# Kitware/SMQTK-Indexing

Hardware: AMD Instinct MI355X
Metric: queries/sec, exact brute-force l2 kNN k=100 over 10000000x128 float32 (recall@100 = 1.0 by construction); scan HBM GB/s vs 8 TB/s peak (higher is better)
Workload: dtype f32 results (distances bit-identical to numpy float32); filter arithmetic int8 MFMA (i32 accumulation, measured per-row error bound), exact re-rank f32

## Files before the change

### smqtk_indexing_amd/csrc/sq_dense_i8.hpp

```cpp
#pragma once
#include "sq_dense_i8_policy.hpp"
#include "sq_dense_scan.hpp"

namespace sq {

typedef int i32x4 __attribute__((ext_vector_type(4)));
typedef int i32x16 __attribute__((ext_vector_type(16)));

template <int KS>
struct I8Geom {
    static constexpr int ROW_BYTES = KS * 32;
    static constexpr int UNIT_ROWS = KS == 4 ? 64 : 32;
    static constexpr int TILES = UNIT_ROWS / 32;
    static constexpr int UNIT_BYTES = UNIT_ROWS * ROW_BYTES;
    static constexpr int SLOT_BYTES = UNIT_BYTES + 256;
    static constexpr int WAVES = KS <= 8 ? 8 : 4;
    static constexpr int NSTAGE = 2;
    static constexpr int PIECES = UNIT_BYTES / 1024;
    static constexpr int SAMPLES_PER_UNIT = 2 * TILES;
};
static constexpr int I8_MAX_ROW_BYTES = 512;
__host__ __device__ constexpr int i8_row_bytes(int d) { return d <= 128 ? 128 : (d <= 256 ? 256 : 512); }
__host__ __device__ constexpr int i8_unit_rows(int row_bytes) { return row_bytes == 128 ? 64 : 32; }

// ... 101 lines not shown
                                                                   const double* __restrict__ nx64, float inv_dx, float dx,
                                                                   signed char* __restrict__ out8, float* __restrict__ nrow,
                                                                   float* __restrict__ r2row, long long row_base, int row_bytes) {
    const int lane = threadIdx.x & 63;
    const long long row = row_base + (long long)blockIdx.x * 4 + (threadIdx.x >> 6);
    if (row >= n_pad) return;
    double e2 = 0.0, r2 = 0.0;
    bool finite = true;
    const double inv_norm = (row < n && nx64) ? 1.0 / sqrt(nx64[row]) : 1.0;
    for (int k0 = 0; k0 < row_bytes; k0 += 64 * EPL) {
        unsigned char q[EPL];
#pragma unroll
        for (int j = 0; j < EPL; ++j) q[j] = 0;
        if (row < n) {
#pragma unroll
            for (int j = 0; j < EPL; ++j) {
                const int k = k0 + EPL * lane + j;
                if (k < d) {
                    const float v = db[row * ld + k];
                    const float xc = i8_element(v, center, k, nx64 != nullptr, inv_norm);
                    if (!(xc == xc) || !(fabsf(xc) < 3.0e38f)) finite = false;
                    float t = rintf(xc * inv_dx);
                    t = fminf(fmaxf(t, -127.f), 127.f);
                    if (!(t == t)) t = 0.f;
                    q[j] = (unsigned char)(signed char)(int)t;
                    const double res = (double)xc - (double)t * (double)dx;
                    e2 += (double)xc * (double)xc;
                    r2 += res * res;
                }
            }
        }
        if (k0 + EPL * lane >= row_bytes) continue;
        unsigned char* dst = reinterpret_cast<unsigned char*>(out8) + row * row_bytes + k0 + EPL * lane;
        if constexpr (EPL == 2) {
            *reinterpret_cast<unsigned short*>(dst) = (unsigned short)(q[0] | (q[1] << 8));
        } else if constexpr (EPL == 4) {
            *reinterpret_cast<u32*>(dst) = (u32)q[0] | ((u32)q[1] << 8) | ((u32)q[2] << 16) | ((u32)q[3] << 24);
        } else {
            uint2 w;
            w.x = (u32)q[0] | ((u32)q[1] << 8) | ((u32)q[2] << 16) | ((u32)q[3] << 24);
            w.y = (u32)q[4] | ((u32)q[5] << 8) | ((u32)q[6] << 16) | ((u32)q[7] << 24);
            *reinterpret_cast<uint2*>(dst) = w;
        }
    }
    finite = __ballot(!finite) == 0ull;
    for (int o = 32; o > 0; o >>= 1) {
        e2 += __shfl_xor(e2, o);
        r2 += __shfl_xor(r2, o);
    }
    if (lane == 0) {
        float nr = __builtin_inff(), rr = 0.f;
        if (row < n && finite) {
            nr = nx64 ? 0.f : (float)e2;
            if ((double)nr > e2) nr = __uint_as_float(__float_as_uint(nr) - 1u);
            rr = (float)r2;
            if ((double)rr < r2) rr = __uint_as_float(__float_as_uint(rr) + 1u);
        }
        nrow[row] = nr;
        r2row[row] = rr;
    }
}

static __global__ __launch_bounds__(256) void dense8_resid_stats_kernel(const float* __restrict__ r2row, const float* __restrict__ nrow,
                                                                         long long n, double* __restrict__ sum_r2,
                                                                         u32* __restrict__ max_bits) {
    __shared__ double red[4];
    __shared__ float rmax[4], nmax[4];
    double acc = 0.0;
    float m = 0.f, mn = 0.f;
    for (long long i = (long long)blockIdx.x * 256 + threadIdx.x; i < n; i += (long long)gridDim.x * 256) {
        const float nv = nrow[i];
        if (nv < __builtin_inff() && nv > -__builtin_inff()) {
            const float v = r2row[i];
            acc += (double)v;
            m = fmaxf(m, v);
            mn = fmaxf(mn, nv);
        }
    }
    for (int o = 32; o > 0; o >>= 1) {
        acc += __shfl_xor(acc, o);
        m = fmaxf(m, __shfl_xor(m, o));
        mn = fmaxf(mn, __shfl_xor(mn, o));
    }
    if ((threadIdx.x & 63) == 0) {
        red[threadIdx.x >> 6] = acc;
        rmax[threadIdx.x >> 6] = m;
        nmax[threadIdx.x >> 6] = mn;
    }
    __syncthreads();
    if (threadIdx.x == 0) {
        atomicAdd(sum_r2, red[0] + red[1] + red[2] + red[3]);
        atomicMax(max_bits, __float_as_uint(fmaxf(fmaxf(rmax[0], rmax[1]), fmaxf(rmax[2], rmax[3]))));
        atomicMax(max_bits + 1, __float_as_uint(fmaxf(fmaxf(nmax[0], nmax[1]), fmaxf(nmax[2], nmax[3]))));
    }
}

static __global__ __launch_bounds__(256) void dense8_flag_kernel(const float* __restrict__ r2row, float* __restrict__ nrow, long long n,
                                                                  float r2_cut, u32* __restrict__ flagged, long long row_base) {
    const long long i = row_base + (long long)blockIdx.x * 256 + threadIdx.x;
    if (i >= n) return;
    if (nrow[i] < __builtin_inff() && r2row[i] > r2_cut) {
        nrow[i] = -__builtin_inff();
        atomicAdd(flagged, 1u);
    }
}

template <int EPL>
__device__ __forceinline__ void dense8_prep_query_row(const float* __restrict__ qrow, bool real, int d, const float* __restrict__ center,
                                                      double dx, double r_max, double x_max, int cosine,
                                                      signed char* __restrict__ p0, signed char* __restrict__ p1, float2& par_out,
                                                      double& qn2_out) {
    const int l16 = threadIdx.x & 15;
    const float sc = cosine ? -1.f : -2.f;
    float v[EPL][4];
#pragma unroll
    for (int c = 0; c < EPL; ++c)
#pragma unroll
        for (int e = 0; e < 4; ++e) {
            const int t = 64 * c + l16 + 16 * e;
            float raw = 0.f, cen = 0.f;
            if (real && t < d) {
                raw = qrow[t];
                if (center) cen = center[t];
            }
            v[c][e] = (real && t < d) ? (center ? __fsub_rn(raw, cen) : raw) : 0.f;
        }
    auto chunk_sum = [](double x0, double x1, double x2, double x3) __attribute__((always_inline)) {
        double sacc = (x0 + x2) + (x1 + x3);
        for (int o = 8; o > 0; o >>= 1) sacc += __shfl_xor(sacc, o);
        return sacc;
    };
    if (cosine) {
        double nn = 0.0;
#pragma unroll
        for (int c = 0; c < EPL; ++c)
            nn += chunk_sum((double)v[c][0] * (double)v[c][0], (double)v[c][1] * (double)v[c][1], (double)v[c][2] * (double)v[c][2],
                            (double)v[c][3] * (double)v[c][3]);
        const double rn = sqrt(nn);
#pragma unroll
        for (int c = 0; c < EPL; ++c)
#pragma unroll
            for (int e = 0; e < 4; ++e) v[c][e] = (float)((double)v[c][e] / rn);
    }
    double Q = 0.0;
    float mx = 0.f;
#pragma unroll
    for (int c = 0; c < EPL; ++c) {
        Q += chunk_sum((double)v[c][0] * (double)v[c][0], (double)v[c][1] * (double)v[c][1], (double)v[c][2] * (double)v[c][2],
                       (double)v[c][3] * (double)v[c][3]);
#pragma unroll
        for (int e = 0; e < 4; ++e) {
            float m = fabsf(sc * v[c][e]);
            if (!(m == m)) m = __builtin_inff();
            mx = fmaxf(mx, m);
        }
    }
    for (int o = 8; o > 0; o >>= 1) mx = fmaxf(mx, __shfl_xor(mx, o));
    const bool ok = real && mx < 3.0e38f && mx > 0.f;
    const double dq = ok ? (double)mx / 127.0 : 1.0;
    const double inv_dq = 1.0 / dq;
    double r2s = 0.0;
#pragma unroll
    for (int c = 0; c < EPL; ++c) {
        double r2[4];
#pragma unroll
        for (int e = 0; e < 4; ++e) {
            const double w = (double)(sc * v[c][e]);
            const double ws = w * inv_dq;
            float qt8 = 0.f, ql8 = 0.f;
            if (ok) {
                qt8 = fminf(fmaxf(rintf((float)ws), -127.f), 127.f);
                ql8 = fminf(fmaxf(rintf((float)((ws - (double)qt8) * 256.0)), -127.f), 127.f);
            }
            const int t = 64 * c + l16 + 16 * e;
            p0[t] = (signed char)(int)qt8;
            p1[t] = (signed char)(int)ql8;
            const double res = w - ((double)qt8 + (double)ql8 * 0.00390625) * dq;
            r2[e] = res * res;
        }
        r2s += chunk_sum(r2[0], r2[1], r2[2], r2[3]);
    }
    const double rq = sqrt(r2s) * (1.0 + 1e-9);
    const double unit = dx * dq;
    const double xr = x_max + r_max, qn = sqrt(Q), wn = (cosine ? 1.0 : 2.0) * qn;
    double e = r_max * wn + xr * rq + 4.0 * 5.9604644775390625e-08 * (xr * (wn + rq) + x_max * x_max);
    e *= 1.0 + 1e-6;
    float ef = (float)e;
    if ((double)ef < e) ef = __uint_as_float(__float_as_uint(ef) + 1u);
    if (!ok && real) ef = __builtin_inff();
    par_out = make_float2((float)unit, real ? ef : 0.f);
    qn2_out = real ? Q : 0.0;
}

template <int EPL>
static __global__ __launch_bounds__(64) void dense8_prep_queries_kernel(const float* __restrict__ q, int nq, int d,
                                                                         const float* __restrict__ center, double dx, double r_max,
                                                                         double x_max, signed char* __restrict__ qs8,
                                                                         float2* __restrict__ par, double* __restrict__ qn2,
                                                                         float* __restrict__ thr, u32* __restrict__ cnt,
                                                                         u32* __restrict__ oflag, float* __restrict__ q_al, int ldq,
                                                                         const DenseCallPtrs* __restrict__ ind, int cosine, int plane_rows) {
    constexpr int row_bytes = EPL * 64;
    if (ind) q = ind->q;
    const int qi = blockIdx.x * 4 + (threadIdx.x >> 4), t = threadIdx.x & 15;
    if (t == 0) {
        thr[qi] = qi < nq ? -__builtin_inff() : __builtin_nanf("");
        cnt[qi] = 0u;
        if (qi == 0) *oflag = 0u;
    }
    if (qi < nq)
        for (int i = t; i < ldq; i += 16) q_al[(long long)qi * ldq + i] = i < d ? q[(long long)qi * d + i] : 0.f;
    float2 pr;
    double Q;
    dense8_prep_query_row<EPL>(q + (long long)qi * d, qi < nq, d, center, dx, r_max, x_max, cosine,
                               qs8 + (long long)qi * row_bytes, qs8 + (long long)(plane_rows + qi) * row_bytes, pr, Q);
    if (t == 0) {
        par[qi] = pr;
        qn2[qi] = Q;
    }
}

struct Dense8ThrPost {
    const float2* par;
    const double* qn2;
    __device__ __forceinline__ void prologue(int, double*) const {}
    __device__ __forceinline__ float operator()(int q, float t) const {
        if (!(t < __builtin_inff())) return t;
        if (!(par[q].y < __builtin_inff())) return __builtin_nanf("");
        const double tt = (double)t + 2.0 * (double)par[q].y + 4e-6 * fabs((double)t + qn2[q]);
        float r = (float)tt;
        if ((double)r < tt) r = __uint_as_float(__float_as_uint(r) + (r >= 0.f ? 1 : -1));
        return r;
    }
};

struct Dense8ScanArgs {
    const signed char* scan8;
    const float* nrow;
    long long n;
    long long n_units;
    const signed char* qs8;
    const float2* par;
    const float* thr;
    uint2* wave_out;
    u32* wave_cnt;
    u32 wave_cap;
    float* sample_out;
    long long ns;
    long long unit_step;
    long long n_sel;
    int nrb;
    int nt;
    long long nt_from_row;
    int nqt;
    int plane_rows;
    int debug;
    float* wave_score;
    u32* hist;
};

template <int KS>
__device__ __forceinline__ int i8_swz(int c, int r) {
    if constexpr (KS == 4) return c ^ ((r >> 1) & 7);
    return (c & ~15) | ((c & 15) ^ (r & 15));
}

enum { I8_EMIT = 0, I8_SAMPLE = 1, I8_LANEMIN = 2, I8_EMIT_H = 3 };

static constexpr int I8_HIST_BINS = 64;
static constexpr int I8_CNT_SHIFT = 5;
static constexpr int I8_HIST_WORDS = TILE_ROWS * I8_HIST_BINS + (TILE_ROWS << I8_CNT_SHIFT);

template <int WAVES>
__device__ __forceinline__ void dense8_hist_flush(u32* lds_hist, u32* __restrict__ ghist) {
    constexpr int PER = TILE_ROWS * I8_HIST_BINS / WAVES;
    const int lane = threadIdx.x & 63;
    const int wave = __builtin_amdgcn_readfirstlane(threadIdx.x >> 6);
#pragma unroll
    for (int i = 0; i < PER / 64; ++i) {
        const int b = wave * PER + i * 64 + lane;
        const u32 v = __hip_atomic_exchange(lds_hist + b, 0u, __ATOMIC_RELAXED, __HIP_MEMORY_SCOPE_WORKGROUP);
        if (v) __hip_atomic_fetch_add(ghist + b, v, __ATOMIC_RELAXED, __HIP_MEMORY_SCOPE_AGENT);
    }
}

template <int KS, int MODE>
__device__ __forceinline__ void dense8_stream(const Dense8ScanArgs& a, unsigned char* smem, const i32x4 (&bq)[KS], const i32x4 (&bl)[KS],
                                              float unit_lo, float thr_l, u32& wcount, float& smin, u32* lds_ticket,
                                              float inv_w_l = 0.f, u32* lds_hist = nullptr) {
    using G = I8Geom<KS>;
    constexpr bool SAMPLE = MODE == I8_SAMPLE || MODE == I8_LANEMIN;
    const int lane = threadIdx.x & 63;
    const int wave = __builtin_amdgcn_readfirstlane(threadIdx.x >> 6);
    const int r31 = lane & 31, h = lane >> 5;
    const u32 lds_base = (u32)(uintptr_t)smem;
    const u32 ring_base = lds_base + (u32)wave * (G::NSTAGE * G::SLOT_BYTES);
    const unsigned char* ring_ptr = smem + wave * (G::NSTAGE * G::SLOT_BYTES);
    const long long wave_id = (long long)blockIdx.x * G::WAVES + wave;
    const long long nwaves = (long long)a.nrb * G::WAVES;
    uint2* wout = a.wave_out + wave_id * a.wave_cap;
    float* wsc = MODE == I8_EMIT_H ? a.wave_score + wave_id * a.wave_cap : nullptr;
    u32* hist_l = MODE == I8_EMIT_H ? lds_hist + r31 * I8_HIST_BINS : nullptr;

    const long long wg_first = (long long)blockIdx.x * G::WAVES;
    auto take_unit = [&]() __attribute__((always_inline)) -> long long {
        u32 t = 0;
        if (lane == 0) t = __hip_atomic_fetch_add(lds_ticket, 1u, __ATOMIC_RELAXED, __HIP_MEMORY_SCOPE_WORKGROUP);
        t = (u32)__builtin_amdgcn_readfirstlane((int)t);
        const long long u = wg_first + (long long)(t % G::WAVES) + (long long)(t / G::WAVES) * nwaves;
        return u < a.n_sel ? u : -1ll;
    };
    const long long my_units = wave_id < a.n_sel ? (a.n_sel - wave_id + nwaves - 1) / nwaves : 0;
    u32 voff[G::PIECES];
#pragma unroll
    for (int j = 0; j < G::PIECES; ++j) {
        const int lin = j * 1024 + lane * 16;
        const int r = lin / G::ROW_BYTES, cpos = (lin % G::ROW_BYTES) >> 4;
        voff[j] = (u32)(r * G::ROW_BYTES + i8_swz<KS>(cpos, r) * 16);
    }
    const u32 voff_n = (u32)lane * 4u;
    static_assert(G::NSTAGE == 2, "two ring slots: the units in flight are sel_even / sel_odd");
    long long issued = 0, sel_even = -1, sel_odd = -1;
    bool more = true;
    auto issue_next = [&]() __attribute__((always_inline)) {
        if (!more) return;
        const long long sel = take_unit();
        if (sel < 0) {
            more = false;
            return;
        }
        if (issued & 1) sel_odd = sel; else sel_even = sel;
        const long long unit_idx = sel * a.unit_step;
        const long long row0 = unit_idx * G::UNIT_ROWS;
        const u32 dst = ring_base + (u32)(issued % G::NSTAGE) * G::SLOT_BYTES;
        const unsigned char* base = reinterpret_cast<const unsigned char*>(a.scan8) + row0 * G::ROW_BYTES;
#pragma unroll
        for (int j = 0; j < G::PIECES; ++j) {
            if (a.nt && row0 >= a.nt_from_row)
                glds16<true>(base, voff[j], dst + (u32)j * 1024);
            else
                glds16<false>(base, voff[j], dst + (u32)j * 1024);
        }
        glds4(a.nrow + row0, voff_n, dst + G::UNIT_BYTES);
        ++issued;
    };
    for (int p = 0; p < G::NSTAGE; ++p) issue_next();
    const int flush_every = (int)(my_units >> 3) > 0 ? (int)(my_units >> 3) : 1;
    int to_flush = flush_every;

    for (long long it = 0; it < issued; ++it) {
        const long long sel = (it & 1) ? sel_odd : sel_even;
        const long long unit_idx = sel * a.unit_step;
        const long long row0 = unit_idx * G::UNIT_ROWS;
        wait_units_in_flight<G::NSTAGE, G::PIECES + 1>((int)(issued - it - 1));
        const unsigned char* sl = ring_ptr + (it % G::NSTAGE) * G::SLOT_BYTES;
        constexpr int KH = KS == 16 ? 8 : KS;
        i32x4 av[G::TILES][KH];
        f32x4 nr[G::TILES][4];
#pragma unroll
        for (int t = 0; t < G::TILES; ++t) {
            const int r = 32 * t + r31;
#pragma unroll
            for (int s = 0; s < KH; ++s)
                av[t][s] = *reinterpret_cast<const i32x4*>(sl + r * G::ROW_BYTES + i8_swz<KS>(2 * s + h, r) * 16);
#pragma unroll
            for (int c = 0; c < 4; ++c) nr[t][c] = *reinterpret_cast<const f32x4*>(sl + G::UNIT_BYTES + (32 * t + 8 * c + 4 * h) * 4);
        }
        asm volatile("s_waitcnt lgkmcnt(0)" ::: "memory");
        if constexpr (KS != 16) issue_next();
#pragma unroll
        for (int t = 0; t < G::TILES; ++t) {
            i32x16 acc, acl;
#pragma unroll
            for (int i = 0; i < 16; ++i) acc[i] = acl[i] = 0;
#pragma unroll
            for (int s = 0; s < KH; ++s) {
                acc = __builtin_amdgcn_mfma_i32_32x32x32_i8(av[t][s], bq[s], acc, 0, 0, 0);
                acl = __builtin_amdgcn_mfma_i32_32x32x32_i8(av[t][s], bl[s], acl, 0, 0, 0);
            }
            if constexpr (KS == 16) {
#pragma unroll
                for (int s = 0; s < KH; ++s)
                    av[t][s] = *reinterpret_cast<const i32x4*>(sl + r31 * G::ROW_BYTES + i8_swz<KS>(2 * (KH + s) + h, r31) * 16);
                asm volatile("s_waitcnt lgkmcnt(0)" ::: "memory");
                issue_next();
#pragma unroll
                for (int s = 0; s < KH; ++s) {
                    acc = __builtin_amdgcn_mfma_i32_32x32x32_i8(av[t][s], bq[KH + s], acc, 0, 0, 0);
                    acl = __builtin_amdgcn_mfma_i32_32x32x32_i8(av[t][s], bl[KH + s], acl, 0, 0, 0);
                }
            }
            if (a.debug & 1024) {
                if (acc[0] == 0x7fffffff && acl[5] == 0x7ffffffe) wcount += 1;
                continue;
            }
            float sc[16];
#pragma unroll
            for (int i = 0; i < 16; ++i) {
                float nv = nr[t][i >> 2][i & 3];
                if constexpr (SAMPLE) nv = nv == -__builtin_inff() ? __builtin_inff() : nv;
                sc[i] = __fmaf_rn((float)((acc[i] << 8) + acl[i]), unit_lo, nv);
            }
            float m = sc[0];
#pragma unroll
            for (int i = 1; i < 16; ++i) m = fminf(m, sc[i]);
            if constexpr (MODE == I8_LANEMIN) {
                smin = fminf(smin, m);
            } else if constexpr (MODE == I8_SAMPLE) {
                a.sample_out[(long long)r31 * a.ns + sel * G::SAMPLES_PER_UNIT + t * 2 + h] = m;
            } else {
                const u64 hit = __ballot(m <= thr_l);
                if (hit != 0) {
                    u32 mask = 0;
#pragma unroll
                    for (int i = 0; i < 16; ++i) mask |= (sc[i] <= thr_l ? 1u : 0u) << i;
                    const u64 bal = __ballot(mask != 0);
                    if (mask) {
                        const u32 pos = wcount + __builtin_amdgcn_mbcnt_hi((u32)(bal >> 32), __builtin_amdgcn_mbcnt_lo((u32)bal, 0u));
                        if (pos < a.wave_cap) {
                            wout[pos] = make_uint2((u32)(row0 + 32 * t + 4 * h), (mask << 16) | (u32)r31);
                            if constexpr (MODE == I8_EMIT_H) wsc[pos] = m;
                        }
                        if constexpr (MODE == I8_EMIT_H) {
                            if (m > -__builtin_inff()) {
                                const int bin = min((int)((thr_l - m) * inv_w_l), I8_HIST_BINS - 1);
                                __hip_atomic_fetch_add(hist_l + bin, 1u, __ATOMIC_RELAXED, __HIP_MEMORY_SCOPE_WORKGROUP);
                            }
                        }
                    }
                    wcount += (u32)__popcll(bal);
                }
            }
        }
        if constexpr (MODE == I8_EMIT_H) {
            if (--to_flush == 0) {
                to_flush = flush_every;
                dense8_hist_flush<G::WAVES>(lds_hist, a.hist);
            }
        }
    }
}

template <int KS>
__device__ __forceinline__ void dense8_load_planes(const signed char* planes, i32x4 (&bq)[KS], i32x4 (&bl)[KS]) {
    using G = I8Geom<KS>;
    const int lane = threadIdx.x & 63, r31 = lane & 31, h = lane >> 5;
#pragma unroll
    for (int s = 0; s < KS; ++s) {
        bq[s] = *reinterpret_cast<const i32x4*>(planes + r31 * G::ROW_BYTES + (2 * s + h) * 16);
        bl[s] = *reinterpret_cast<const i32x4*>(planes + (TILE_ROWS + r31) * G::ROW_BYTES + (2 * s + h) * 16);
    }
#pragma unroll
    for (int s = 0; s < KS; ++s) asm volatile("" : "+v"(bq[s]), "+v"(bl[s]));
}

template <int KS, bool SAMPLE>
__global__ __launch_bounds__(I8Geom<KS>::WAVES * 64, KS == 16 ? 1 : 2) void dense8_scan_kernel(Dense8ScanArgs a) {
    using G = I8Geom<KS>;
    extern __shared__ __attribute__((aligned(16))) unsigned char smem[];
    const int lane = threadIdx.x & 63;
    const int wave = __builtin_amdgcn_readfirstlane(threadIdx.x >> 6);
    const int r31 = lane & 31;
    i32x4 bq[KS], bl[KS];
    dense8_load_planes<KS>(a.qs8, bq, bl);
    float unit_lo = a.par[r31].x * 0.00390625f;
    float thr_l = SAMPLE ? 0.f : a.thr[r31];
    asm volatile("" : "+v"(unit_lo), "+v"(thr_l));
    u32 wcount = 0;
    float smin = 0.f;
    __shared__ u32 s_unit_ticket;
    if (threadIdx.x == 0) s_unit_ticket = 0u;
    __syncthreads();
    dense8_stream<KS, SAMPLE ? I8_SAMPLE : I8_EMIT>(a, smem, bq, bl, unit_lo, thr_l, wcount, smin, &s_unit_ticket);
    if constexpr (!SAMPLE) {
        if (lane == 0) {
            const long long wave_id = (long long)blockIdx.x * G::WAVES + wave;
            a.wave_cnt[2 * wave_id] = wcount;
            a.wave_cnt[2 * wave_id + 1] = 0u;
        }
    }
}


struct Dense8HeadArgs {
    Dense8ScanArgs s;
    const float* q;
    int nq, d;
    const float* center;
    double dx, r_max, x_max;
    int cosine;
    double* qn2;
    u32* cnt;
    u32* oflag;
    float* q_al;
    int ldq;
    const DenseCallPtrs* ind;
    float* lane_min;
    int keep;
    int kk;
};

template <int VM, int NQ>
__device__ __forceinline__ void wave_kth_smallest(const float* __restrict__ vals, long long stride, int M, int k, float (&out)[NQ]) {
    const int lane = threadIdx.x & 63;
    constexpr u32 KINF = 0xff800000u;
    u32 key[NQ][VM];
    u32 prefix[NQ];
    u32 xall = 0u;
#pragma unroll
    for (int n = 0; n < NQ; ++n) {
        u32 kmin = KINF, kmax = 0u;
#pragma unroll
        for (int j = 0; j < VM; ++j) {
            const int i = j * 64 + lane;
            u32 kv = ordered_f32(vals[n * stride + (i < M ? i : 0)]);
            kv = (i < M && kv < KINF) ? kv : KINF;
            key[n][j] = kv;
            kmin = kv < kmin ? kv : kmin;
            kmax = kv > kmax ? kv : kmax;
        }
        for (int o = 32; o > 0; o >>= 1) {
            const u32 a = (u32)__shfl_xor((int)kmin, o), b = (u32)__shfl_xor((int)kmax, o);
            kmin = a < kmin ? a : kmin;
            kmax = b > kmax ? b : kmax;
        }
        prefix[n] = __builtin_amdgcn_readfirstlane(kmin);
        xall |= __builtin_amdgcn_readfirstlane(kmin ^ kmax);
    }
    if (xall != 0u) {
        const int top = 31 - __clz((int)xall);
#pragma unroll
        for (int n = 0; n < NQ; ++n) prefix[n] &= ~((2u << top) - 1u);
        for (int b = top; b >= 0; --b) {
#pragma unroll
            for (int n = 0; n < NQ; ++n) {
                const u32 cand = prefix[n] | ((1u << b) - 1u);
                u32 c = 0;
#pragma unroll
                for (int j = 0; j < VM; ++j) c += (u32)__popcll(__ballot(key[n][j] <= cand));
                if (c < (u32)k) prefix[n] |= 1u << b;
            }
        }
    }
#pragma unroll
    for (int n = 0; n < NQ; ++n) {
        float r = unordered_f32(prefix[n]);
        if (prefix[n] >= KINF) {
            u32 c = 0;
#pragma unroll
            for (int j = 0; j < VM; ++j) c += (u32)__popcll(__ballot(key[n][j] < KINF));
            if (c < (u32)k) r = __builtin_inff();
        }
        out[n] = r;
    }
}

template <int KS>
__global__ __launch_bounds__(I8Geom<KS>::WAVES * 64, KS == 16 ? 1 : 2) void dense8_head_kernel(Dense8HeadArgs ha) {
    using G = I8Geom<KS>;
    constexpr int VB = G::WAVES * 2;
    extern __shared__ __attribute__((aligned(16))) unsigned char smem[];
    __shared__ float2 s_par[TILE_ROWS];
    __shared__ double s_qn2[TILE_ROWS];
    __shared__ float s_lm[TILE_ROWS][16];
    __shared__ u32 s_ticket, s_unit_ticket;
    if (threadIdx.x == 0) s_unit_ticket = 0u;
    const Dense8ScanArgs& a = ha.s;
    const int lane = threadIdx.x & 63;
    const int wave = __builtin_amdgcn_readfirstlane(threadIdx.x >> 6);
    const int r31 = lane & 31, h = lane >> 5;
    const float* q = ha.ind ? ha.ind->q : ha.q;
    const bool first = blockIdx.x == 0;
    signed char* planes = reinterpret_cast<signed char*>(smem);
#pragma unroll
    for (int rnd = 0; rnd < TILE_ROWS / (4 * G::WAVES); ++rnd) {
        const int qi = rnd * 4 * G::WAVES + wave * 4 + (lane >> 4);
        float2 pr;
        double Q;
        dense8_prep_query_row<KS / 2>(q + (long long)qi * ha.d, qi < ha.nq, ha.d, ha.center, ha.dx, ha.r_max, ha.x_max, ha.cosine,
                                      planes + qi * G::ROW_BYTES, planes + (TILE_ROWS + qi) * G::ROW_BYTES, pr, Q);
        if ((lane & 15) == 0) {
            s_par[qi] = pr;
            s_qn2[qi] = Q;
        }
        if (first) {
            if ((lane & 15) == 0) {
                const_cast<float2*>(a.par)[qi] = pr;
                ha.qn2[qi] = Q;
                ha.cnt[qi << I8_CNT_SHIFT] = 0u;
                if (qi == 0) ha.oflag[0] = 0u;
            }
            if (qi < ha.nq)
                for (int i = lane & 15; i < ha.ldq; i += 16) ha.q_al[(long long)qi * ha.ldq + i] = i < ha.d ? q[(long long)qi * ha.d + i] : 0.f;
        }
    }
    __syncthreads();
    i32x4 bq[KS], bl[KS];
    dense8_load_planes<KS>(planes, bq, bl);
    float unit_lo = s_par[r31].x * 0.00390625f;
    asm volatile("" : "+v"(unit_lo));
    if (first) {
        signed char* gp = const_cast<signed char*>(a.qs8);
        for (int i = threadIdx.x; i < 2 * TILE_ROWS * G::ROW_BYTES / 16; i += G::WAVES * 64)
            reinterpret_cast<uint4*>(gp)[i] = reinterpret_cast<const uint4*>(planes)[i];
        for (int i = threadIdx.x; i < I8_HIST_WORDS; i += G::WAVES * 64) a.hist[i] = 0u;
    }
    asm volatile("s_waitcnt vmcnt(0) lgkmcnt(0)" ::: "memory");
    __syncthreads();
    u32 wcount = 0;
    float smin = __builtin_inff();
    if (!(a.debug & 4096)) dense8_stream<KS, I8_LANEMIN>(a, smem, bq, bl, unit_lo, 0.f, wcount, smin, &s_unit_ticket);
    s_lm[r31][(wave * 2 + h) & 15] = smin;
    if (VB < 16 && wave == 0 && h == 0)
        for (int i = VB; i < 16; ++i) s_lm[r31][i] = __builtin_inff();
    __syncthreads();
    const int nb = (int)gridDim.x, keep = ha.keep, M = nb * keep;
#pragma unroll
    for (int rnd = 0; rnd < TILE_ROWS / (4 * G::WAVES); ++rnd) {
        const int qi = rnd * 4 * G::WAVES + wave * 4 + (lane >> 4), l16 = lane & 15;
        float v = s_lm[qi][l16];
#pragma unroll
        for (int kk2 = 2; kk2 <= 16; kk2 <<= 1)
#pragma unroll
            for (int j = kk2 >> 1; j > 0; j >>= 1) {
                const float o = __shfl_xor(v, j);
                const bool up = (l16 & kk2) == 0, lower = (l16 & j) == 0;
                v = (lower == up) ? fminf(v, o) : fmaxf(v, o);
            }
        if (l16 < keep) ha.lane_min[(long long)qi * M + (long long)blockIdx.x * keep + l16] = v;
    }
    asm volatile("s_waitcnt vmcnt(0)" ::: "memory");
    __syncthreads();
    if (threadIdx.x == 0) {
        __threadfence();
        const u32 t = atomicAdd(&ha.oflag[1], 1u);
        if (t == gridDim.x - 1) {
            __threadfence();
            ha.oflag[1] = 0u;
        }
        s_ticket = t;
    }
    __syncthreads();
    if (s_ticket != gridDim.x - 1) return;
    float* thr = const_cast<float*>(a.thr);
    const Dense8ThrPost post{s_par, s_qn2};
#pragma unroll
    for (int rnd = 0; rnd < TILE_ROWS / (4 * G::WAVES); ++rnd) {
        const int q0 = rnd * 4 * G::WAVES + wave * 4;
        float ts[4] = {-__builtin_inff(), -__builtin_inff(), -__builtin_inff(), -__builtin_inff()};
        if (q0 < ha.nq && !(a.debug & 2048)) {
            const float* v = ha.lane_min + (long long)q0 * M;
            if (M <= 256)
                wave_kth_smallest<4, 4>(v, M, M, ha.kk, ts);
            else if (M <= 512)
                wave_kth_smallest<8, 4>(v, M, M, ha.kk, ts);
            else if (M <= 1024)
                wave_kth_smallest<16, 4>(v, M, M, ha.kk, ts);
            else {
#pragma unroll
                for (int j = 0; j < 4; ++j) {
                    float one[1];
                    wave_kth_smallest<32, 1>(v + (long long)j * M, M, M, ha.kk, one);
                    ts[j] = one[0];
                }
            }
        }
#pragma unroll
        for (int j = 0; j < 4; ++j) {
            const float t = q0 + j < ha.nq ? post(q0 + j, ts[j]) : __builtin_nanf("");
            if (lane == 0) thr[q0 + j] = t;
        }
    }
}

struct Dense8TailArgs {
    const float* db;
    long long ld;
    int d;
    const float* q_al;
    int ldq, nq;
    void* keys;
    u32* cnt;
    u32 cap;
    u32* overflow;
    const double* nx64;
    const double* nq64;
    int debug;
    const double* qn2;
    int kk;
    int tighten;
    long long* clk;
};
static constexpr int I8_TAIL_QROWS_BYTES = 32 * (156 + 4) * 4;
static constexpr int I8_TAIL_LIST = 2048;
static constexpr int I8_TAIL_RERANK_BYTES = I8_TAIL_QROWS_BYTES + 3 * RERANK_MAX_GROUP * 4 + 8 * 32 * RERANK_STAGE_STRIDE * 4;
static constexpr int I8_TAIL_LDS_BYTES = I8_TAIL_RERANK_BYTES + I8_TAIL_LIST * 8 + TILE_ROWS * 4 + 16;

template <int KS, bool COSINE>
__global__ __launch_bounds__(I8Geom<KS>::WAVES * 64, KS == 16 ? 1 : 2) void dense8_body_kernel(Dense8ScanArgs a, Dense8TailArgs ta) {
    using G = I8Geom<KS>;
    static_assert(I8_TAIL_LDS_BYTES <= G::WAVES * G::NSTAGE * G::SLOT_BYTES, "the re-rank works in the ring's LDS");
    extern __shared__ __attribute__((aligned(16))) unsigned char smem[];
    __shared__ u32 s_hist8[TILE_ROWS * I8_HIST_BINS];
    __shared__ u32 s_wcnt[G::WAVES];
    __shared__ u32 s_unit_ticket;
    __shared__ float s_thr1[TILE_ROWS], s_eq[TILE_ROWS];
    __shared__ double s_qn2b[TILE_ROWS];
    __shared__ float2 s_parb[TILE_ROWS];
    if (threadIdx.x == 0) s_unit_ticket = 0u;
    if (threadIdx.x < TILE_ROWS) {
        s_thr1[threadIdx.x] = a.thr[threadIdx.x];
        s_parb[threadIdx.x] = a.par[threadIdx.x];
        s_eq[threadIdx.x] = a.par[threadIdx.x].y;
        s_qn2b[threadIdx.x] = ta.qn2[threadIdx.x];
    }
    const int lane = threadIdx.x & 63;
    const int wave = __builtin_amdgcn_readfirstlane(threadIdx.x >> 6);
    const int r31 = lane & 31;
    for (int i = threadIdx.x; i < TILE_ROWS * I8_HIST_BINS; i += G::WAVES * 64) s_hist8[i] = 0u;
    long long* clk = ta.clk ? ta.clk + (long long)blockIdx.x * 8 : nullptr;
    if (clk && threadIdx.x == 0) {
        clk[0] = (long long)wall_clock64();
        clk[1] = 0x7fffffffffffffffll;
    }
    __syncthreads();
    i32x4 bq[KS], bl[KS];
    dense8_load_planes<KS>(a.qs8, bq, bl);
    float unit_lo = a.par[r31].x * 0.00390625f;
    float thr_l = a.thr[r31];
    const float eq_l = a.par[r31].y;
    float inv_w_l = (eq_l > 0.f && eq_l < __builtin_inff()) ? 2.f / eq_l : 0.f;
    if (!(inv_w_l < 3.0e38f)) inv_w_l = 0.f;
    asm volatile("" : "+v"(unit_lo), "+v"(thr_l), "+v"(inv_w_l));
    u32 wcount = 0;
    float smin = 0.f;
    dense8_stream<KS, I8_EMIT_H>(a, smem, bq, bl, unit_lo, thr_l, wcount, smin, &s_unit_ticket, inv_w_l, s_hist8);
    const long long w0 = (long long)blockIdx.x * G::WAVES;
    if (lane == 0) {
        a.wave_cnt[2 * (w0 + wave)] = wcount;
        a.wave_cnt[2 * (w0 + wave) + 1] = 0u;
        s_wcnt[wave] = wcount;
        if (clk) atomicMin((unsigned long long*)(clk + 1), (unsigned long long)wall_clock64());
// ... 225 lines not shown
```

### smqtk_indexing_amd/csrc/sq_dma.hpp

```cpp
#pragma once
#include "sq_common.hpp"

namespace sq {

__device__ __forceinline__ const void* uniform_ptr(const void* p) {
    const u64 v = (u64)(uintptr_t)p;
    const u32 lo = __builtin_amdgcn_readfirstlane((u32)v), hi = __builtin_amdgcn_readfirstlane((u32)(v >> 32));
    return (const void*)(uintptr_t)(((u64)hi << 32) | lo);
}
template <bool NT = false>
__device__ __forceinline__ void glds16(const void* gbase_uniform, u32 voff, u32 lds_dst) {
    u32 keep;
    if constexpr (NT)
        asm volatile(
            "s_mov_b32 %0, m0\n\t"
            "s_mov_b32 m0, %3\n\t"
            "s_nop 0\n\t"
            "global_load_lds_dwordx4 %1, %2 nt\n\t"
            "s_mov_b32 m0, %0"
            : "=&s"(keep)
            : "v"(voff), "s"(uniform_ptr(gbase_uniform)), "s"(__builtin_amdgcn_readfirstlane(lds_dst))
            : "memory");
    else
        asm volatile(
            "s_mov_b32 %0, m0\n\t"
            "s_mov_b32 m0, %3\n\t"
            "s_nop 0\n\t"
            "global_load_lds_dwordx4 %1, %2\n\t"
            "s_mov_b32 m0, %0"
            : "=&s"(keep)
            : "v"(voff), "s"(uniform_ptr(gbase_uniform)), "s"(__builtin_amdgcn_readfirstlane(lds_dst))
            : "memory");
}
__device__ __forceinline__ void glds4(const void* gbase_uniform, u32 voff, u32 lds_dst) {
    u32 keep;
    asm volatile(
        "s_mov_b32 %0, m0\n\t"
        "s_mov_b32 m0, %3\n\t"
        "s_nop 0\n\t"
        "global_load_lds_dword %1, %2\n\t"
        "s_mov_b32 m0, %0"
        : "=&s"(keep)
        : "v"(voff), "s"(uniform_ptr(gbase_uniform)), "s"(__builtin_amdgcn_readfirstlane(lds_dst))
        : "memory");
}

__device__ __forceinline__ void glds_set_m0(u32 lds_dst) {
    asm volatile("s_mov_b32 m0, %0\n\ts_nop 0" ::"s"(__builtin_amdgcn_readfirstlane(lds_dst)) : "memory");
}
template <int OFF, bool NT = false>
__device__ __forceinline__ void glds16_m0(const void* gbase_uniform, u32 voff) {
    static_assert(OFF >= -4096 && OFF <= 4095, "13-bit signed instruction offset");
    if constexpr (NT)
        asm volatile("global_load_lds_dwordx4 %0, %1 offset:%2 nt" ::"v"(voff), "s"(uniform_ptr(gbase_uniform)), "n"(OFF) : "memory");
    else
        asm volatile("global_load_lds_dwordx4 %0, %1 offset:%2" ::"v"(voff), "s"(uniform_ptr(gbase_uniform)), "n"(OFF) : "memory");
}
template <int OFF>
__device__ __forceinline__ void glds4_m0(const void* gbase_uniform, u32 voff) {
    static_assert(OFF >= -4096 && OFF <= 4095, "13-bit signed instruction offset");
    asm volatile("global_load_lds_dword %0, %1 offset:%2" ::"v"(voff), "s"(uniform_ptr(gbase_uniform)), "n"(OFF) : "memory");
}
template <int N, int J = 0, class F>
__device__ __forceinline__ void static_for_one(int j, F&& f) {
    if constexpr (J < N) {
        if (j == J)
            f(std::integral_constant<int, J>{});
        else
            static_for_one<N, J + 1>(j, f);
    }
}

template <int N>
__device__ __forceinline__ void wait_vmcnt() {
    asm volatile("s_waitcnt vmcnt(%0)" ::"n"(N) : "memory");
}

template <int NSTAGE, int PER>
__device__ __forceinline__ void wait_units_in_flight(int units) {
    if constexpr (NSTAGE >= 4) {
        if (units >= 3) {
            wait_vmcnt<3 * PER>();
            return;
        }
    }
    if constexpr (NSTAGE >= 3) {
        if (units == 2) {
            wait_vmcnt<2 * PER>();
            return;
        }
    }
    if (units == 1)
        wait_vmcnt<PER>();
    else
        wait_vmcnt<0>();
}

__device__ __forceinline__ void store_u64_counted(u64* p, u64 v) {
    asm volatile("global_store_dwordx2 %0, %1, off" ::"v"(p), "v"(v) : "memory");
}

template <int PER, int S, int EMAX, int U, int E>
__device__ __forceinline__ void wait_ops_rec(int units, int epis) {
    if (units == U && epis == E) {
        wait_vmcnt<(U * PER + E * S < 63 ? U * PER + E * S : 63)>();
        return;
    }
    if constexpr (E > 0)
        wait_ops_rec<PER, S, EMAX, U, E - 1>(units, epis);
    else if constexpr (U > 0)
        wait_ops_rec<PER, S, EMAX, U - 1, EMAX>(units, epis);
    else
        wait_vmcnt<0>();
}
template <int NSTAGE, int PER, int S>
__device__ __forceinline__ void wait_ops_in_flight(int units, int epis) {
    wait_ops_rec<PER, S, NSTAGE, NSTAGE - 1, NSTAGE>(units, epis);
}

}
```

Baseline: 144,900.

## Batch unit DMA issue into single asm blocks and simplify ring-slot bookkeeping

Result: faster. 150,100 (median of 6 runs) (+3.6%).

```diff
diff --git a/smqtk_indexing_amd/csrc/sq_dense_i8.hpp b/smqtk_indexing_amd/csrc/sq_dense_i8.hpp
--- a/smqtk_indexing_amd/csrc/sq_dense_i8.hpp
+++ b/smqtk_indexing_amd/csrc/sq_dense_i8.hpp
@@ -427,58 +427,68 @@
     float* wsc = MODE == I8_EMIT_H ? a.wave_score + wave_id * a.wave_cap : nullptr;
     u32* hist_l = MODE == I8_EMIT_H ? lds_hist + r31 * I8_HIST_BINS : nullptr;
 
-    const long long wg_first = (long long)blockIdx.x * G::WAVES;
-    auto take_unit = [&]() __attribute__((always_inline)) -> long long {
-        u32 t = 0;
-        if (lane == 0) t = __hip_atomic_fetch_add(lds_ticket, 1u, __ATOMIC_RELAXED, __HIP_MEMORY_SCOPE_WORKGROUP);
-        t = (u32)__builtin_amdgcn_readfirstlane((int)t);
-        const long long u = wg_first + (long long)(t % G::WAVES) + (long long)(t / G::WAVES) * nwaves;
-        return u < a.n_sel ? u : -1ll;
+    using U = unsigned long long;
+    constexpr U NONE = ~(U)0;
+    static_assert((G::WAVES & (G::WAVES - 1)) == 0, "ticket -> unit by shift and mask");
+    const U wg_first = (U)blockIdx.x * G::WAVES, nwaves_u = (U)nwaves, n_sel = (U)a.n_sel, unit_step = (U)a.unit_step;
+    const u32 ticket_addr = (u32)(uintptr_t)lds_ticket;
+    auto take_unit = [&]() __attribute__((always_inline)) -> U {
+        const u32 t = lds_ticket_take(ticket_addr);
+        const U u = wg_first + (U)(t & (u32)(G::WAVES - 1)) + (U)(t / G::WAVES) * nwaves_u;
+        return u < n_sel ? u : NONE;
     };
     const long long my_units = wave_id < a.n_sel ? (a.n_sel - wave_id + nwaves - 1) / nwaves : 0;
-    u32 voff[G::PIECES];
+    u32 voff_s[G::PIECES];
 #pragma unroll
     for (int j = 0; j < G::PIECES; ++j) {
         const int lin = j * 1024 + lane * 16;
         const int r = lin / G::ROW_BYTES, cpos = (lin % G::ROW_BYTES) >> 4;
-        voff[j] = (u32)(r * G::ROW_BYTES + i8_swz<KS>(cpos, r) * 16);
+        voff_s[j] = (u32)(r * G::ROW_BYTES + i8_swz<KS>(cpos, r) * 16) + 4096u - (u32)j * 1024u;
     }
     const u32 voff_n = (u32)lane * 4u;
-    static_assert(G::NSTAGE == 2, "two ring slots: the units in flight are sel_even / sel_odd");
-    long long issued = 0, sel_even = -1, sel_odd = -1;
-    bool more = true;
-    auto issue_next = [&]() __attribute__((always_inline)) {
-        if (!more) return;
-        const long long sel = take_unit();
-        if (sel < 0) {
-            more = false;
-            return;
-        }
-        if (issued & 1) sel_odd = sel; else sel_even = sel;
-        const long long unit_idx = sel * a.unit_step;
-        const long long row0 = unit_idx * G::UNIT_ROWS;
-        const u32 dst = ring_base + (u32)(issued % G::NSTAGE) * G::SLOT_BYTES;
-        const unsigned char* base = reinterpret_cast<const unsigned char*>(a.scan8) + row0 * G::ROW_BYTES;
-#pragma unroll
-        for (int j = 0; j < G::PIECES; ++j) {
-            if (a.nt && row0 >= a.nt_from_row)
-                glds16<true>(base, voff[j], dst + (u32)j * 1024);
-            else
-                glds16<false>(base, voff[j], dst + (u32)j * 1024);
-        }
-        glds4(a.nrow + row0, voff_n, dst + G::UNIT_BYTES);
-        ++issued;
+    static_assert(G::NSTAGE == 2, "two ring slots: the unit consumed and the unit in flight");
+    static_assert(G::PIECES == 8 || G::PIECES == 16, "a unit is one or two glds_unit8 statements");
+    U nt_from_unit = NONE;
+    if (a.nt) {
+        const long long f = a.nt_from_row / G::UNIT_ROWS + (a.nt_from_row % G::UNIT_ROWS != 0 ? 1 : 0);
+        nt_from_unit = (U)f;
+    }
+    auto issue_unit = [&](U u, u32 slot_off) __attribute__((always_inline)) {
+        const U unit_idx = u * unit_step;
+        const unsigned char* base = reinterpret_cast<const unsigned char*>(a.scan8) + (unsigned long long)unit_idx * G::UNIT_BYTES;
+        const float* terms = a.nrow + (unsigned long long)unit_idx * G::UNIT_ROWS;
+        const u32 dst = ring_base + slot_off;
+        if (unit_idx >= nt_from_unit) {
+            if constexpr (G::PIECES == 16) glds_unit8<true, false>(base, voff_s, dst);
+            glds_unit8<true, true>(base + (G::PIECES - 8) * 1024, voff_s + (G::PIECES - 8), dst + (G::PIECES - 8) * 1024, terms, voff_n,
+                                   dst + G::UNIT_BYTES);
+        } else {
+            if constexpr (G::PIECES == 16) glds_unit8<false, false>(base, voff_s, dst);
+            glds_unit8<false, true>(base + (G::PIECES - 8) * 1024, voff_s + (G::PIECES - 8), dst + (G::PIECES - 8) * 1024, terms, voff_n,
+                                    dst + G::UNIT_BYTES);
+        }
     };
-    for (int p = 0; p < G::NSTAGE; ++p) issue_next();
+    U u_cur = take_unit(), u_nxt = NONE;
+    bool more = u_cur != NONE;
+    if (more) {
+        issue_unit(u_cur, 0u);
+        u_nxt = take_unit();
+        more = u_nxt != NONE;
+        if (more) issue_unit(u_nxt, (u32)G::SLOT_BYTES);
+    }
     const int flush_every = (int)(my_units >> 3) > 0 ? (int)(my_units >> 3) : 1;
     int to_flush = flush_every;
 
-    for (long long it = 0; it < issued; ++it) {
-        const long long sel = (it & 1) ? sel_odd : sel_even;
-        const long long unit_idx = sel * a.unit_step;
-        const long long row0 = unit_idx * G::UNIT_ROWS;
-        wait_units_in_flight<G::NSTAGE, G::PIECES + 1>((int)(issued - it - 1));
-        const unsigned char* sl = ring_ptr + (it % G::NSTAGE) * G::SLOT_BYTES;
+    u32 slot_off = 0u;
+    while (u_cur != NONE) {
+        const U sel = u_cur;
+        const u32 row0 = (u32)(sel * unit_step) * (u32)G::UNIT_ROWS;
+        if (u_nxt != NONE)
+            wait_vmcnt<G::PIECES + 1>();
+        else
+            wait_vmcnt<0>();
+        const unsigned char* sl = ring_ptr + slot_off;
+        U u_new = NONE;
         constexpr int KH = KS == 16 ? 8 : KS;
         i32x4 av[G::TILES][KH];
         f32x4 nr[G::TILES][4];
@@ -492,7 +502,15 @@
             for (int c = 0; c < 4; ++c) nr[t][c] = *reinterpret_cast<const f32x4*>(sl + G::UNIT_BYTES + (32 * t + 8 * c + 4 * h) * 4);
         }
         asm volatile("s_waitcnt lgkmcnt(0)" ::: "memory");
-        if constexpr (KS != 16) issue_next();
+        auto refill = [&]() __attribute__((always_inline)) {
+            if (!more) return;
+            u_new = take_unit();
+            if (u_new != NONE)
+                issue_unit(u_new, slot_off);
+            else
+                more = false;
+        };
+        if constexpr (KS != 16) refill();
 #pragma unroll
         for (int t = 0; t < G::TILES; ++t) {
             i32x16 acc, acl;
@@ -508,7 +526,7 @@
                 for (int s = 0; s < KH; ++s)
                     av[t][s] = *reinterpret_cast<const i32x4*>(sl + r31 * G::ROW_BYTES + i8_swz<KS>(2 * (KH + s) + h, r31) * 16);
                 asm volatile("s_waitcnt lgkmcnt(0)" ::: "memory");
-                issue_next();
+                refill();
 #pragma unroll
                 for (int s = 0; s < KH; ++s) {
                     acc = __builtin_amdgcn_mfma_i32_32x32x32_i8(av[t][s], bq[KH + s], acc, 0, 0, 0);
@@ -519,7 +537,7 @@
                 if (acc[0] == 0x7fffffff && acl[5] == 0x7ffffffe) wcount += 1;
                 continue;
             }
-            float sc[16];
+            f32x16 sc;
 #pragma unroll
             for (int i = 0; i < 16; ++i) {
                 float nv = nr[t][i >> 2][i & 3];
@@ -532,16 +550,13 @@
             if constexpr (MODE == I8_LANEMIN) {
                 smin = fminf(smin, m);
             } else if constexpr (MODE == I8_SAMPLE) {
-                a.sample_out[(long long)r31 * a.ns + sel * G::SAMPLES_PER_UNIT + t * 2 + h] = m;
+                a.sample_out[(long long)r31 * a.ns + (long long)sel * G::SAMPLES_PER_UNIT + t * 2 + h] = m;
             } else {
                 const u64 hit = __ballot(m <= thr_l);
                 if (hit != 0) {
-                    u32 mask = 0;
-#pragma unroll
-                    for (int i = 0; i < 16; ++i) mask |= (sc[i] <= thr_l ? 1u : 0u) << i;
-                    const u64 bal = __ballot(mask != 0);
+                    const u32 mask = le_mask16(sc, thr_l);
                     if (mask) {
-                        const u32 pos = wcount + __builtin_amdgcn_mbcnt_hi((u32)(bal >> 32), __builtin_amdgcn_mbcnt_lo((u32)bal, 0u));
+                        const u32 pos = wcount + __builtin_amdgcn_mbcnt_hi((u32)(hit >> 32), __builtin_amdgcn_mbcnt_lo((u32)hit, 0u));
                         if (pos < a.wave_cap) {
                             wout[pos] = make_uint2((u32)(row0 + 32 * t + 4 * h), (mask << 16) | (u32)r31);
                             if constexpr (MODE == I8_EMIT_H) wsc[pos] = m;
@@ -553,7 +568,7 @@
                             }
                         }
                     }
-                    wcount += (u32)__popcll(bal);
+                    wcount += (u32)__popcll(hit);
                 }
             }
         }
@@ -563,6 +578,9 @@
                 dense8_hist_flush<G::WAVES>(lds_hist, a.hist);
             }
         }
+        u_cur = u_nxt;
+        u_nxt = u_new;
+        slot_off = (u32)G::SLOT_BYTES - slot_off;
     }
 }
 
diff --git a/smqtk_indexing_amd/csrc/sq_dma.hpp b/smqtk_indexing_amd/csrc/sq_dma.hpp
--- a/smqtk_indexing_amd/csrc/sq_dma.hpp
+++ b/smqtk_indexing_amd/csrc/sq_dma.hpp
@@ -61,6 +61,65 @@
     static_assert(OFF >= -4096 && OFF <= 4095, "13-bit signed instruction offset");
     asm volatile("global_load_lds_dword %0, %1 offset:%2" ::"v"(voff), "s"(uniform_ptr(gbase_uniform)), "n"(OFF) : "memory");
 }
+#define SQ_GLDS16X8(NT_)                                              \
+    "s_mov_b32 m0, %9\n\t"                                            \
+    "s_nop 0\n\t"                                                     \
+    "global_load_lds_dwordx4 %0, %8 offset:-4096" NT_ "\n\t"          \
+    "global_load_lds_dwordx4 %1, %8 offset:-3072" NT_ "\n\t"          \
+    "global_load_lds_dwordx4 %2, %8 offset:-2048" NT_ "\n\t"          \
+    "global_load_lds_dwordx4 %3, %8 offset:-1024" NT_ "\n\t"          \
+    "global_load_lds_dwordx4 %4, %8" NT_ "\n\t"                       \
+    "global_load_lds_dwordx4 %5, %8 offset:1024" NT_ "\n\t"           \
+    "global_load_lds_dwordx4 %6, %8 offset:2048" NT_ "\n\t"           \
+    "global_load_lds_dwordx4 %7, %8 offset:3072" NT_
+#define SQ_GLDS4_TERMS           \
+    "\n\ts_mov_b32 m0, %10\n\t"  \
+    "s_nop 0\n\t"                \
+    "global_load_lds_dword %11, %12"
+template <bool NT, bool TERMS>
+__device__ __forceinline__ void glds_unit8(const void* gbase_uniform, const u32* voff_s, u32 lds_dst, const void* terms_uniform = nullptr,
+                                           u32 voff_terms = 0, u32 lds_terms = 0) {
+    const u32 m0a = __builtin_amdgcn_readfirstlane(lds_dst + 4096u), m0b = __builtin_amdgcn_readfirstlane(lds_terms);
+    const void* gb = uniform_ptr(gbase_uniform);
+    if constexpr (TERMS) {
+        const void* tb = uniform_ptr(terms_uniform);
+        if constexpr (NT)
+            asm volatile(SQ_GLDS16X8(" nt") SQ_GLDS4_TERMS ::"v"(voff_s[0]), "v"(voff_s[1]), "v"(voff_s[2]), "v"(voff_s[3]), "v"(voff_s[4]),
+                         "v"(voff_s[5]), "v"(voff_s[6]), "v"(voff_s[7]), "s"(gb), "s"(m0a), "s"(m0b), "v"(voff_terms), "s"(tb)
+                         : "memory");
+        else
+            asm volatile(SQ_GLDS16X8("") SQ_GLDS4_TERMS ::"v"(voff_s[0]), "v"(voff_s[1]), "v"(voff_s[2]), "v"(voff_s[3]), "v"(voff_s[4]),
+                         "v"(voff_s[5]), "v"(voff_s[6]), "v"(voff_s[7]), "s"(gb), "s"(m0a), "s"(m0b), "v"(voff_terms), "s"(tb)
+                         : "memory");
+    } else {
+        if constexpr (NT)
+            asm volatile(SQ_GLDS16X8(" nt")::"v"(voff_s[0]), "v"(voff_s[1]), "v"(voff_s[2]), "v"(voff_s[3]), "v"(voff_s[4]), "v"(voff_s[5]),
+                         "v"(voff_s[6]), "v"(voff_s[7]), "s"(gb), "s"(m0a)
+                         : "memory");
+        else
+            asm volatile(SQ_GLDS16X8("")::"v"(voff_s[0]), "v"(voff_s[1]), "v"(voff_s[2]), "v"(voff_s[3]), "v"(voff_s[4]), "v"(voff_s[5]),
+                         "v"(voff_s[6]), "v"(voff_s[7]), "s"(gb), "s"(m0a)
+                         : "memory");
+    }
+}
+#undef SQ_GLDS16X8
+#undef SQ_GLDS4_TERMS
+
+__device__ __forceinline__ u32 lds_ticket_take(u32 lds_addr) {
+    u32 tv;
+    u64 keep;
+    asm volatile(
+        "s_mov_b64 %1, exec\n\t"
+        "s_mov_b64 exec, 1\n\t"
+        "ds_add_rtn_u32 %0, %2, %3\n\t"
+        "s_mov_b64 exec, %1\n\t"
+        "s_waitcnt lgkmcnt(0)"
+        : "=&v"(tv), "=&s"(keep)
+        : "v"(lds_addr), "v"(1u)
+        : "memory");
+    return (u32)__builtin_amdgcn_readfirstlane((int)tv);
+}
+
 template <int N, int J = 0, class F>
 __device__ __forceinline__ void static_for_one(int j, F&& f) {
     if constexpr (J < N) {
```
